# ESandML/SSL4GIE

Measured on AMD Instinct MI355X. Metric: images/sec/GPU (fwd+bwd) ViT-B 224² bs=256 at 1/2/4/8 MI355X; % MFMA peak, higher is better.
Workload: dtype bf16; 1 GPU; ViT-B MAE pretrain (mae_vit_base_patch16, norm_pix_loss, mask 0.75) fwd+bwd+grad-allreduce+AdamW, 224x224 synthetic N(0,1) images resident in HBM; batch_per_gpu=256, global_batch=256, parallelism=dp1, optimizer=AdamW(0.9,0.95) wd 0.05 (ssl4gie_amd.optim.ArenaAdamW)

## Files before the change

### include/ssl4gie_hip.h

```cpp
#ifndef SSL4GIE_HIP_H
#define SSL4GIE_HIP_H
#include <stddef.h>
#include <stdint.h>
#ifdef __cplusplus
extern "C" {
#endif

#define SSL4GIE_F32 0
#define SSL4GIE_BF16 1
#define SSL4GIE_EARG 1000
#define SSL4GIE_EPEER 1001

int ssl4gie_abi_version(void);

int ssl4gie_layernorm_fwd(const float* x, const float* gamma, const float* beta, void* y,
                          int y_dtype, float* mean, float* rstd, int rows, int cols, float eps,
                          void* stream);
size_t ssl4gie_layernorm_bwd_workspace_bytes(int rows, int cols);
int ssl4gie_layernorm_bwd(const void* dy, int dy_dtype, const float* x, const float* gamma,
                          const float* mean, const float* rstd, const float* dres, float* dx,
                          void* dx_lp, int lp_dtype, float* dgamma, float* dbeta, int accumulate,
                          float* workspace, int rows, int cols, void* stream);

size_t ssl4gie_colsum_workspace_bytes(int rows, int cols);
// ... 246 lines not shown
int ssl4gie_maxpool3x3s2_fwd(const void* x, void* y, unsigned char* arg, int dtype, int B, int H,
                             int W, int C, void* stream);
int ssl4gie_maxpool3x3s2_bwd(const void* dy, const unsigned char* arg, void* dx, int dtype, int B,
                             int H, int W, int C, void* stream);
int ssl4gie_bn_maxpool3x3s2_fwd(const void* x, const float* coef, int relu, void* y, unsigned char* arg,
                                int dtype, int B, int H, int W, int C, void* stream);
int ssl4gie_avgpool_fwd(const void* x, float* y, int dtype, int B, int HW, int C, void* stream);
int ssl4gie_avgpool_bwd(const float* dy, void* dx, int dtype, int B, int HW, int C, void* stream);

int ssl4gie_adamw_arena(float* p, const float* g, float* m, float* v, const long long* seg_start,
                        const float* seg_lr, const float* seg_wd, int S, float beta1, float beta2,
                        float eps, int step, long long n, void* stream);
int ssl4gie_adamw_arena_lp(float* p, const float* g, float* m, float* v, const long long* seg_start,
                           const float* seg_lr, const float* seg_wd, int S, float beta1, float beta2,
                           float eps, int step, long long n, void* lp_bf16, void* stream);
int ssl4gie_adamw_arena_range(float* p, const float* g, float* m, float* v, const long long* seg_start,
                              const float* seg_lr, const float* seg_wd, int S, float beta1, float beta2,
                              float eps, int step, long long lo, long long hi, void* lp_bf16,
                              void* stream);
size_t ssl4gie_grad_norm_workspace_bytes(void);
int ssl4gie_grad_norm_arena(const float* g, const long long* seg_start, const float* seg_mask, int S,
                            float inv_scale, float max_norm, void* workspace, float* ctl, long long n,
                            void* stream);
int ssl4gie_grad_scale_arena(float* g, const long long* seg_start, const float* seg_mask, int S,
                             const float* ctl, long long n, void* stream);
int ssl4gie_adamw_arena_range_ctl(float* p, const float* g, float* m, float* v, const long long* seg_start,
                                  const float* seg_lr, const float* seg_wd, int S, float beta1, float beta2,
                                  float eps, int* applied, long long lo, long long hi, void* lp_bf16,
                                  const float* ctl, int skip_nonfinite, int advance, void* stream);
size_t ssl4gie_lars_workspace_bytes(int S);
// ... 157 lines not shown
```

### ssl4gie_amd/_lib.py

```python
from __future__ import annotations

import ctypes as C
import os

_HERE = os.path.dirname(os.path.abspath(__file__))
LIB_PATH = os.path.join(_HERE, "libssl4gie_hip.so")
ABI_VERSION = 12

PROF_KINDS = 7

F32, BF16 = 0, 1
BWD_ACCUMULATE, BWD_NO_JOIN = 1, 4
EPI_NONE, EPI_BIAS, EPI_BIAS_GELU, EPI_BIAS_RESIDUAL, EPI_DGELU, EPI_BIAS_GELU_GRAD, EPI_MUL_AUX, \
    EPI_RELU_MASK_AUX, EPI_ADD_AUX, EPI_AFFINE_AUX_RELU = range(10)
BN_FROM_X, BN_FROM_PARTIALS, BN_FROM_STATS, BN_FROM_COEF = range(4)
FILTER_BILINEAR, FILTER_BICUBIC = 0, 1
TGT_U8, TGT_U16, TGT_F32 = range(3)
DET_MAP_MAX_PER_IMAGE, DET_MAP_CLASSES, DET_MAP_CHUNK = 1024, 256, 256
NMS_MAX_PER_SEGMENT = 4096
PRED_I64 = 2
ERASE_CONST, ERASE_RAND, ERASE_PIXEL = range(3)
BN_MASK_NONE, BN_MASK_Y, BN_MASK_X, BN_MASK_BITS = range(4)

vp, i32, i64, f32, sz = C.c_void_p, C.c_int, C.c_longlong, C.c_float, C.c_size_t
# ... 104 lines not shown
    "ssl4gie_bn_workspace_bytes": (sz, [i64, i32]),
    "ssl4gie_bn_fwd": (i32, [i32, vp, vp, i32, vp, vp, vp, vp, vp, vp, vp, vp, vp, vp, f32, f32, i32, vp, i32, i64, i32,
                             vp]),
    "ssl4gie_bn_stats": (i32, [vp, vp, i32, vp, vp, vp, i32, i64, i32, vp]),
    "ssl4gie_bn_bwd": (i32, [vp, i32, vp, vp, vp, vp, vp, vp, vp, vp, vp, vp, i32, vp, i32, i64, i32, vp]),
    "ssl4gie_bn_bwd_reduce": (i32, [vp, i32, vp, vp, vp, vp, vp, vp, vp, vp, vp, i32, i64, i32, vp]),
    "ssl4gie_bn_bwd_apply": (i32, [vp, i32, vp, vp, vp, vp, vp, vp, vp, f32, vp, vp, i32, i64, i32, vp]),
    "ssl4gie_ema_update": (i32, [vp, vp, f32, i64, vp]),
    "ssl4gie_maxpool3x3s2_fwd": (i32, [vp, vp, vp, i32, i32, i32, i32, i32, vp]),
    "ssl4gie_bn_maxpool3x3s2_fwd": (i32, [vp, vp, i32, vp, vp, i32, i32, i32, i32, i32, vp]),
    "ssl4gie_maxpool3x3s2_bwd": (i32, [vp, vp, vp, i32, i32, i32, i32, i32, vp]),
    "ssl4gie_avgpool_fwd": (i32, [vp, vp, i32, i32, i32, i32, vp]),
    "ssl4gie_avgpool_bwd": (i32, [vp, vp, i32, i32, i32, i32, vp]),
    "ssl4gie_adamw_arena": (i32, [vp, vp, vp, vp, vp, vp, vp, i32, f32, f32, f32, i32, i64, vp]),
    "ssl4gie_adamw_arena_lp": (i32, [vp, vp, vp, vp, vp, vp, vp, i32, f32, f32, f32, i32, i64, vp, vp]),
    "ssl4gie_adamw_arena_range": (i32, [vp, vp, vp, vp, vp, vp, vp, i32, f32, f32, f32, i32, i64, i64, vp, vp]),
    "ssl4gie_adamw_arena_range_ctl": (i32, [vp, vp, vp, vp, vp, vp, vp, i32, f32, f32, f32, vp, i64, i64, vp, vp,
                                            i32, i32, vp]),
    "ssl4gie_grad_norm_workspace_bytes": (sz, []),
    "ssl4gie_grad_norm_arena": (i32, [vp, vp, vp, i32, f32, f32, vp, vp, i64, vp]),
    "ssl4gie_grad_scale_arena": (i32, [vp, vp, vp, i32, vp, i64, vp]),
    "ssl4gie_lars_workspace_bytes": (sz, [i32]),
    "ssl4gie_lars_arena": (i32, [vp, vp, vp, vp, vp, vp, vp, i32, f32, f32, vp, i64, vp]),
    "ssl4gie_normalize_u8": (i32, [vp, vp, C.POINTER(C.c_float), C.POINTER(C.c_float), i32, i32, i32, vp]),
    "ssl4gie_view_sample_u8": (i32, [vp, i64, i32, i32, vp, vp, vp, vp, i32, i32, i32, C.POINTER(C.c_float),
                                     C.POINTER(C.c_float), vp]),
    "ssl4gie_quantize_u8": (i32, [vp, vp, i32, i32, vp]),
    "ssl4gie_randaug_layer_workspace_bytes": (sz, [i32]),
    "ssl4gie_randaug_layer": (i32, [vp, vp, vp, vp, vp, C.POINTER(C.c_ubyte), vp, i32, i32, vp]),
    "ssl4gie_normalize_erase_u8": (i32, [vp, vp, C.POINTER(C.c_float), C.POINTER(C.c_float), vp, i32, C.c_ulonglong, i32,
# ... 129 lines not shown
```

### ssl4gie_amd/csrc/engine.hip

```cpp
#include "common.h"
#include "ssl4gie_hip.h"

#include <string.h>
#include <stdlib.h>
#include <mutex>
#include "prof.h"
#include "internal.h"

extern "C" int ssl4gie_abi_version(void) { return 12; }

namespace { extern int g_wgrad_stream; }
extern "C" int ssl4gie_set_wgrad_stream(int on) {
    g_wgrad_stream = on ? 1 : 0;
    return 0;
}

ProfState g_prof = {false, 0, 0, nullptr, nullptr, nullptr};

extern "C" int ssl4gie_prof_begin(int max_launches) {
    REQUIRE(max_launches > 0 && !g_prof.ev);
    g_prof.ev = (hipEvent_t*)calloc((size_t)2 * max_launches, sizeof(hipEvent_t));
    g_prof.kind = (int*)calloc(max_launches, sizeof(int));
    g_prof.flops = (double*)calloc(max_launches, sizeof(double));
    REQUIRE(g_prof.ev && g_prof.kind && g_prof.flops);
// ... 292 lines not shown
    RC(linear_bwd_data(du, w->wfc1, w->wfc1_t, T, F, D, dt, e, stream));
    const bool ln_side = ss != nullptr;
    RC(ssl4gie_layernorm_bwd(dh, dt, a->xmid, w->ln2_g, a->mean2, a->rstd2, dx_out, dxmid,
                             (dt == SSL4GIE_F32 || s_attn) ? nullptr : dxmid_lp, dt, ln_side ? nullptr : g->ln2_g,
                             ln_side ? nullptr : g->ln2_b, accumulate, ln_ws, T, D, stream));
    if (s_attn) {
        RC(ssl4gie_drop_path_scale_cast(dxmid, s_attn, ws + P.dys_mid, dt, d->B, per_sample, stream));
        dxmid_lp = ws + P.dys_mid;
    }
    memset(&e, 0, sizeof(e));
    e.C = dattn; e.ldc = D; e.dtype_c = dt; e.epilogue = SSL4GIE_EPI_NONE;
    RC(linear_bwd_data(dxmid_lp, w->wproj, w->wproj_t, T, D, D, dt, e, stream));
    RC(ssl4gie_attn_bwd(a->qkv, a->attn, dattn, a->lse, dqkv, dt, d->B, d->N, d->H, D / d->H,
                        ws + L.attn_ws, stream));
    RC(fork());
    if (ln_side)
        RC(ssl4gie_internal_ln_reduce(ln_ws, g->ln2_g, g->ln2_b, T, D, accumulate, (hipStream_t)wst));
    wg = wgrad_desc(D, D, T, dxmid_lp, a->attn, g->wproj, g->bproj, dt, accumulate);
    wg2 = wgrad_desc(3 * D, D, T, dqkv, a->h1, g->wqkv, g->bqkv, dt, accumulate);
    RC(ssl4gie_gemm_tn_pair(&wg, &wg2, gws, L.gemm_ws_bytes, wst));
    memset(&e, 0, sizeof(e));
    e.C = dh; e.ldc = D; e.dtype_c = dt; e.epilogue = SSL4GIE_EPI_NONE;
    RC(linear_bwd_data(dqkv, w->wqkv, w->wqkv_t, T, 3 * D, D, dt, e, stream));
    RC(ssl4gie_layernorm_bwd(dh, dt, x_in, w->ln1_g, a->mean1, a->rstd1, dxmid, dx_in,
                             dt == SSL4GIE_F32 ? nullptr : dx_in_lp, dt, ln_side ? nullptr : g->ln1_g,
                             ln_side ? nullptr : g->ln1_b, accumulate, ln_side ? ln_ws1 : ln_ws, T, D, stream));
    if (ln_side) {
        RC(fork());
        RC(ssl4gie_internal_ln_reduce(ln_ws1, g->ln1_g, g->ln1_b, T, D, accumulate, ss->s));
    }
    if (ss && no_join) {
        HIP_RET(hipEventRecord(ss->ev[5 + slot], ss->s));
        ss->slot_used[slot] = true;
    } else if (ss) {
        HIP_RET(hipEventRecord(ss->ev[4], ss->s));
// ... 32 lines not shown
```

### ssl4gie_amd/csrc/gemm.hip

```cpp
#include "gemm_internal.h"

#include <mutex>
#include "prof.h"
#include <stdlib.h>

struct GemmArgs {
    int M, N, K, batch2;
    const void* A;
    long long sAm, sAk, sAb1, sAb2;
    const void* B;
    long long sBk, sBn, sBb1, sBb2;
    void* C;
    long long ldc, sCb1, sCb2;
    EpiArgs e;
};

template <typename TC, bool VEC, bool FAST = false>
DEVI void epi_store4(const EpiArgs& e, TC* __restrict__ C, long long ldc, int m, int n, int M,
                     int N, f32x4 acc) {
    if (m >= M || n >= N) return;
    const size_t off = (size_t)m * ldc + n;
    if (VEC) {
        f32x4 v = acc * e.alpha;
        switch (e.mode) {
// ... 583 lines not shown
        compute(cur);
    }

    float* out = (splits == 1) ? C : slabs + (size_t)split * M * N;
    const long long ldo = (splits == 1) ? ldc : N;
    EpiArgs es = e;
    if (splits != 1) { es.mode = SSL4GIE_EPI_NONE; es.accumulate = 0; es.alpha = 1.f; }
    epi_wave_tile<float, SSL4GIE_EPI_NONE>(es, out, ldo, m0 + wm, n0 + wn, M, N, acc, lane);
}

__global__ void slab_reduce_kernel(const float* __restrict__ slabs, float* __restrict__ C,
                                   long long ldc, int M, int N, int splits, float alpha,
                                   int accumulate, const float* __restrict__ cs_part,
                                   float* __restrict__ cs_out, unsigned c_blocks) {
    if (blockIdx.x >= c_blocks) {
        const int m = (blockIdx.x - c_blocks) * blockDim.x + threadIdx.x;
        if (m < M) {
            float s = 0.f;
            for (int k = 0; k < splits; ++k) s += cs_part[(size_t)k * M + m];
            cs_out[m] = accumulate ? cs_out[m] + s : s;
        }
        return;
    }
    const size_t i4 = (size_t)blockIdx.x * blockDim.x + threadIdx.x;
    const size_t total4 = (size_t)M * N / 4;
    if (i4 >= total4) return;
    const size_t idx = i4 * 4;
    const int m = (int)(idx / N), n = (int)(idx % N);
    f32x4 s = ld4(slabs + idx);
    int k = 1;
    for (; k + 3 < splits; k += 4) {
        const f32x4 a = ld4(slabs + (size_t)k * M * N + idx), b = ld4(slabs + (size_t)(k + 1) * M * N + idx);
        const f32x4 c2 = ld4(slabs + (size_t)(k + 2) * M * N + idx), d2 = ld4(slabs + (size_t)(k + 3) * M * N + idx);
        s += a; s += b; s += c2; s += d2;
    }
    for (; k < splits; ++k) s += ld4(slabs + (size_t)k * M * N + idx);
    s *= alpha;
    float* c = C + (size_t)m * ldc + n;
    if (accumulate) s += ld4(c);
    st4(c, s);
}

template <int G>
__global__ __launch_bounds__(64 * G) void slab_reduce_wide_kernel(const float* __restrict__ slabs,
                                                                  float* __restrict__ C, long long ldc, int M, int N,
                                                                  int splits, float alpha, int accumulate) {
    __shared__ f32x4 part[G - 1][64];
    const int c = threadIdx.x & 63, g = threadIdx.x >> 6;
    const size_t i4 = (size_t)blockIdx.x * 64 + c;
    const size_t total4 = (size_t)M * N / 4;
    const bool ok = i4 < total4;
    const size_t idx = i4 * 4, slab = (size_t)M * N;
    f32x4 s = {0, 0, 0, 0};
    if (ok)
    {
// ... 270 lines not shown
};
static TnManyPlan tn_many_plan(const ssl4gie_gemm_desc* ds, int n, int splits) {
    TnManyPlan p;
    size_t o = 0;
    for (int i = 0; i < n; ++i) {
        p.slab_off[i] = o;
        if (splits > 1) o += align256((size_t)splits * ds[i].M * ds[i].N * sizeof(float));
    }
    for (int i = 0; i < n; ++i) {
        p.cs_off[i] = o;
        if (splits > 1 && ds[i].colsum_a) o += align256((size_t)splits * ds[i].M * sizeof(float));
    }
    p.total = o;
    return p;
}
static int tn_many_run(const ssl4gie_gemm_desc* ds, int n, int splits, void* workspace, size_t workspace_bytes,
                       hipStream_t st) {
    for (int i = 0; i < n; ++i) {
        REQUIRE(ds[i].A && ds[i].B && ds[i].C);
        REQUIRE(!ds[i].colsum_a || ds[i].sAk >= ds[i].M);
    }
    const TnManyPlan p = tn_many_plan(ds, n, splits);
    REQUIRE(p.total == 0 || (workspace && workspace_bytes >= p.total));
    char* ws = (char*)workspace;
    float* slabs[TN_GROUP_MAX];
    float* cs[TN_GROUP_MAX];
    double flops = 0;
    for (int i = 0; i < n; ++i) {
        slabs[i] = splits > 1 ? (float*)(ws + p.slab_off[i]) : nullptr;
        cs[i] = (splits > 1 && ds[i].colsum_a) ? (float*)(ws + p.cs_off[i]) : nullptr;
        flops += 2.0 * ds[i].K * (double)ds[i].M * ds[i].N;
    }
    {
        ProfScope prof(PROF_GEMM_TN, flops, st);
        const int rc = ssl4gie_internal_tn256_launch(ds, n, splits, slabs, cs, st);
        if (rc) return rc;
    }
    for (int i = 0; splits > 1 && i < n; ++i) {
        const ssl4gie_gemm_desc* d = &ds[i];
        const int rc = launch_slab_reduce(slabs[i], (float*)d->C, d->ldc, d->M, d->N, splits, d->alpha, d->accumulate,
                                          cs[i], d->colsum_a, d->colsum_a != nullptr, false, st);
        if (rc) return rc;
    }
    return 0;
}

static bool tn_pair_ok(const ssl4gie_gemm_desc* a, const ssl4gie_gemm_desc* b) {
    return a && b && !nt_ok(a) && !nt_ok(b) && tn_ok(a) && tn_ok(b) && !a->conv && !b->conv &&
           ssl4gie_internal_tn256_ok(a) && ssl4gie_internal_tn256_ok(b) && a->K == b->K &&
           a->accumulate == b->accumulate && a->alpha == 1.f && b->alpha == 1.f &&
           a->N % 4 == 0 && b->N % 4 == 0;
}
extern "C" size_t ssl4gie_gemm_tn_pair_workspace_bytes(const ssl4gie_gemm_desc* a,
                                                       const ssl4gie_gemm_desc* b) {
    if (!a || !b) return 0;
    if (tn_pair_ok(a, b)) {
        const ssl4gie_gemm_desc ds[2] = {*a, *b};
// ... 1 lines not shown
    }
    const size_t wa = ssl4gie_gemm_workspace_bytes(a), wb = ssl4gie_gemm_workspace_bytes(b);
    return wa > wb ? wa : wb;
}
extern "C" int ssl4gie_gemm_tn_pair(const ssl4gie_gemm_desc* a, const ssl4gie_gemm_desc* b,
                                    void* workspace, size_t workspace_bytes, void* stream) {
    REQUIRE(a && b);
    if (!tn_pair_ok(a, b)) {
        const int rc = ssl4gie_gemm(a, workspace, workspace_bytes, stream);
        if (rc) return rc;
        return ssl4gie_gemm(b, workspace, workspace_bytes, stream);
    }
    const ssl4gie_gemm_desc ds[2] = {*a, *b};
    return tn_many_run(ds, 2, ssl4gie_internal_tn256_splits(ds, 2, TN_SPLIT_PAIR), workspace, workspace_bytes,
                       (hipStream_t)stream);
}

static bool tn_group_ok(const ssl4gie_gemm_desc* ds, int n) {
    if (!ds || n < 1 || n > TN_GROUP_MAX) return false;
    for (int i = 0; i < n; ++i) {
        const ssl4gie_gemm_desc* d = &ds[i];
        if (nt_ok(d) || !tn_ok(d) || d->conv || !ssl4gie_internal_tn256_ok(d) || d->K != ds[0].K ||
            d->N % 4 != 0 || d->dtype_c != SSL4GIE_F32)
            return false;
    }
    return true;
}
extern "C" size_t ssl4gie_gemm_tn_group_workspace_bytes(const ssl4gie_gemm_desc* descs, int n) {
    if (!descs || n < 1) return 0;
    if (tn_group_ok(descs, n))
// ... 22 lines not shown
```

### ssl4gie_amd/csrc/internal.h

```cpp
#pragma once
#include <hip/hip_runtime.h>
#include <stddef.h>

int ssl4gie_internal_reduce_partials(const float* partial, float* out, int nparts, int n_out,
                                     size_t stride, int accumulate, hipStream_t st);

int ssl4gie_internal_ln_reduce(const float* workspace, float* dgamma, float* dbeta, int rows, int cols,
                               int accumulate, hipStream_t st);
```

### ssl4gie_amd/csrc/norm.hip

```cpp
#include "common.h"
#include "prof.h"
#include "ssl4gie_hip.h"
#include "internal.h"

int ssl4gie_internal_compute_cus();

#define LN_ROWS_PER_BLOCK 4
#define LN_MAX_VEC 8

template <int NV> DEVI int ln_col(int i, int lane, int cols) {
    const int c = (i * 64 + lane) * 4;
    return (NV <= 4 && i < NV - 1) || c < cols ? c : 0;
}

static constexpr int ln_fwd_per_cu(int nv) { return nv == 1 ? 8 : nv == 2 ? 6 : nv == 3 ? 5 : nv == 4 ? 4 : 2; }
template <typename TY, int NV>
__global__ __launch_bounds__(256, ln_fwd_per_cu(NV)) void ln_fwd_kernel(const float* __restrict__ x,
                                                     const float* __restrict__ gamma,
                                                     const float* __restrict__ beta,
                                                     TY* __restrict__ y, float* __restrict__ mean,
                                                     float* __restrict__ rstd, int rows, int cols,
                                                     float eps) {
    const int lane = threadIdx.x & 63;
    const int stride = gridDim.x * LN_ROWS_PER_BLOCK;
// ... 303 lines not shown
                f32x4 og = ag[i], ob = ab[i];
#pragma unroll
                for (int w = 0; w < 3; ++w)
#pragma unroll
                    for (int j = 0; j < 4; ++j) {
                        og[j] += red[w][(i * 4 + j) * 64 + lane];
                        ob[j] += red[w][(NV * 4 + i * 4 + j) * 64 + lane];
                    }
                st4(pg + c, og);
                st4(pb + c, ob);
            }
        }
    }
}

#define RP_WAVES 16
__global__ __launch_bounds__(64 * RP_WAVES) void reduce_partials_kernel(
    const float* __restrict__ partial, float* __restrict__ out0, float* __restrict__ out1,
    int split, int nparts, int n_out, size_t stride, int accumulate) {
    __shared__ float red[RP_WAVES][64];
    const int lane = threadIdx.x & 63, wave = threadIdx.x >> 6;
    const int c = blockIdx.x * 64 + lane;
    float s0 = 0.f, s1 = 0.f, s2 = 0.f, s3 = 0.f;
    if (c < n_out) {
        int p = wave;
        for (; p + 15 * RP_WAVES < nparts; p += 16 * RP_WAVES) {
            float a[16];
#pragma unroll
            for (int u = 0; u < 16; ++u) a[u] = partial[(size_t)(p + u * RP_WAVES) * stride + c];
#pragma unroll
            for (int u = 0; u < 16; u += 4) { s0 += a[u]; s1 += a[u + 1]; s2 += a[u + 2]; s3 += a[u + 3]; }
        }
        for (; p + 3 * RP_WAVES < nparts; p += 4 * RP_WAVES) {
            s0 += partial[(size_t)p * stride + c];
            s1 += partial[(size_t)(p + RP_WAVES) * stride + c];
            s2 += partial[(size_t)(p + 2 * RP_WAVES) * stride + c];
            s3 += partial[(size_t)(p + 3 * RP_WAVES) * stride + c];
        }
        for (; p < nparts; p += RP_WAVES) s0 += partial[(size_t)p * stride + c];
    }
    red[wave][lane] = (s0 + s1) + (s2 + s3);
    __syncthreads();
    if (wave == 0 && c < n_out) {
        float s = 0.f;
#pragma unroll
        for (int w = 0; w < RP_WAVES; ++w) s += red[w][lane];
        float* o = (c < split) ? out0 + c : out1 + (c - split);
        *o = accumulate ? *o + s : s;
    }
}

template <typename T>
__global__ __launch_bounds__(256) void colsum_partial_kernel(const T* __restrict__ x,
                                                             float* __restrict__ partial,
                                                             int rows, int cols, size_t ld) {
    __shared__ f32x4 red[3][64];
    const int lane = threadIdx.x & 63, wave = threadIdx.x >> 6;
    const int c = (blockIdx.x * 64 + lane) * 4;
    f32x4 acc = {0, 0, 0, 0};
    if (c < cols) {
        for (int r = blockIdx.y * 4 + wave; r < rows; r += gridDim.y * 4) {
            const f32x4 v = ld4(x + (size_t)r * ld + c);
            acc += v;
        }
// ... 144 lines not shown
    }
#undef LN_BWD
#undef LN_BWD_RES
    LAUNCH_CHECK();
    if (dgamma && dbeta) {
        hipLaunchKernelGGL(reduce_partials_kernel, dim3((2 * cols + 63) / 64), dim3(64 * RP_WAVES),
                           0, st, workspace, dgamma, dbeta, cols, nb, 2 * cols, (size_t)2 * cols,
                           accumulate);
        LAUNCH_CHECK();
    }
    return 0;
}

int ssl4gie_internal_ln_reduce(const float* workspace, float* dgamma, float* dbeta, int rows, int cols,
                               int accumulate, hipStream_t st) {
    if (rows == 0 || !dgamma || !dbeta) return 0;
    const int nb = ln_bwd_blocks(rows);
    hipLaunchKernelGGL(reduce_partials_kernel, dim3((2 * cols + 63) / 64), dim3(64 * RP_WAVES), 0, st, workspace,
                       dgamma, dbeta, cols, nb, 2 * cols, (size_t)2 * cols, accumulate);
    LAUNCH_CHECK();
    return 0;
}

static bool colsum_narrow(int cols) { return cols <= 128 && cols % 4 == 0 && ((cols / 4) & (cols / 4 - 1)) == 0; }
static int colsum_parts(int rows, int cols) {
    const int cap = colsum_narrow(cols) ? 2048 : 256;
    int p = (rows + 63) / 64;
    return p < cap ? (p < 1 ? 1 : p) : cap;
}
extern "C" size_t ssl4gie_colsum_workspace_bytes(int rows, int cols) {
    return (size_t)colsum_parts(rows, cols) * cols * sizeof(float);
}
extern "C" int ssl4gie_colsum(const void* x, int dtype, float* out, int accumulate,
                              float* workspace, int rows, int cols, long long ld, void* stream) {
    REQUIRE(x && out && workspace && rows >= 0 && cols > 0 && ld >= cols);
    REQUIRE(dtype == SSL4GIE_F32 || dtype == SSL4GIE_BF16);
// ... 30 lines not shown
```

### ssl4gie_amd/csrc/optim_ops.hip

```cpp
#include "reduce.h"
#include "ssl4gie_hip.h"

namespace {
DEVI int find_seg(const long long* __restrict__ seg_start, int S, long long i) {
    int lo = 0, hi = S;
    while (hi - lo > 1) {
        const int mid = (lo + hi) >> 1;
        if (seg_start[mid] <= i) lo = mid;
        else hi = mid;
    }
    return lo;
}
DEVI int block_seg(const long long* __restrict__ seg_start, int S, long long i, long long block_first) {
    __shared__ int s0;
    if (threadIdx.x == 0) s0 = find_seg(seg_start, S, block_first);
    __syncthreads();
    int s = s0;
    while (s + 1 < S && seg_start[s + 1] <= i) ++s;
    return s;
}
}

template <bool CTL>
__global__ __launch_bounds__(256) void adamw_arena_kernel(
    float* __restrict__ p, const float* __restrict__ g, float* __restrict__ m, float* __restrict__ v,
    const long long* __restrict__ seg_start, const float* __restrict__ seg_lr,
    const float* __restrict__ seg_wd, int S, float b1, float b2, float eps, float bc1, float rsqrt_bc2,
    long long n, bf16_t* __restrict__ lp, long long lo, const float* __restrict__ ctl,
    const int* __restrict__ applied, int skip) {
    __shared__ float bc[2];
    float coef = 1.f;
    if (CTL) {
        if (skip && ctl[2] != 0.f) return;
        coef = ctl[1];
// ... 18 lines not shown
#pragma unroll
    for (int j = 0; j < 4; ++j) {
        float x = pp[j] * (1.f - lr * wd);
        const float mj = b1 * mm[j] + (1.f - b1) * gg[j];
        const float vj = b2 * vv[j] + (1.f - b2) * gg[j] * gg[j];
        x -= step * mj / (sqrtf(vj) * rsqrt_bc2 + eps);
        pp[j] = x; mm[j] = mj; vv[j] = vj;
    }
    st4(p + i, pp);
    st4(m + i, mm);
    st4(v + i, vv);
    if (lp) st4(lp + i, pp);
}
__global__ void adamw_advance_kernel(int* __restrict__ applied, const float* __restrict__ ctl, int skip) {
    if (!(skip && ctl[2] != 0.f)) *applied += 1;
}

#define GN_BLOCKS 2048
__global__ __launch_bounds__(256) void grad_norm_partial_kernel(
    const float* __restrict__ g, const long long* __restrict__ seg_start,
    const float* __restrict__ seg_mask, int S, float inv_scale, long long n, long long per_block,
    double* __restrict__ part_sum, int* __restrict__ part_bad) {
    __shared__ double red[4];
    __shared__ int redb[4];
    f32x4 acc = {0.f, 0.f, 0.f, 0.f};
    unsigned bad = 0;
    const long long lo = (long long)blockIdx.x * per_block;
    const long long hi = lo + per_block < n ? lo + per_block : n;
    long long i = lo + threadIdx.x * 4;
    if (i < hi) {
// ... 212 lines not shown
                                        const float* ctl, long long n, void* stream) {
    REQUIRE(g && seg_start && seg_mask && S > 0 && ctl && n > 0 && n % 4 == 0);
    hipLaunchKernelGGL(grad_scale_kernel, dim3((unsigned)((n / 4 + 255) / 256)), dim3(256), 0,
                       (hipStream_t)stream, g, seg_start, seg_mask, S, ctl, n);
    LAUNCH_CHECK();
    return 0;
}
extern "C" int ssl4gie_adamw_arena_lp(float* p, const float* g, float* m, float* v,
                                      const long long* seg_start, const float* seg_lr,
                                      const float* seg_wd, int S, float beta1, float beta2, float eps,
                                      int step, long long n, void* lp_bf16, void* stream) {
    REQUIRE(n >= 0);
    return ssl4gie_adamw_arena_range(p, g, m, v, seg_start, seg_lr, seg_wd, S, beta1, beta2, eps, step, 0, n,
                                     lp_bf16, stream);
}
extern "C" int ssl4gie_adamw_arena(float* p, const float* g, float* m, float* v,
                                   const long long* seg_start, const float* seg_lr,
                                   const float* seg_wd, int S, float beta1, float beta2, float eps,
                                   int step, long long n, void* stream) {
    return ssl4gie_adamw_arena_lp(p, g, m, v, seg_start, seg_lr, seg_wd, S, beta1, beta2, eps, step, n,
                                  nullptr, stream);
}
extern "C" size_t ssl4gie_lars_workspace_bytes(int S) {
    return ((size_t)S * LARS_PARTS * 2 + S) * sizeof(float);
}
extern "C" int ssl4gie_lars_arena(float* p, const float* g, float* mu, const long long* seg_start,
                                  const float* seg_lr, const float* seg_wd, const float* seg_mat, int S,
                                  float momentum, float trust, float* workspace, long long n,
                                  void* stream) {
    REQUIRE(p && g && mu && seg_start && seg_lr && seg_wd && seg_mat && workspace && S > 0 && S <= 65535 &&
// ... 17 lines not shown
```

### ssl4gie_amd/engine.py

```python
from __future__ import annotations

import ctypes as C
import contextlib
import os
import weakref
from dataclasses import dataclass
from typing import Callable, List, Optional, Sequence

import torch
import torch.nn as nn

from . import _lib, ops
from ._lib import BlockAct, BlockDims, BlockGrads, BlockWeights


def default_dtype():
    v = os.environ.get("SSL4GIE_PRECISION", "bf16").lower()
    return torch.float32 if v in ("fp32", "f32", "float32") else torch.bfloat16


def _align(n, a=256):
    return (n + a - 1) // a * a


# ... 60 lines not shown
        if getattr(self, "_lp_stamp", None) != weights_epoch():
            self._refresh_lp()
        o = self._index[id(p)]
        rows = p.shape[0]
        cols = p.numel() // rows
        return (self._lp[o:o + p.numel()].view(rows, cols), self._lpt[o:o + p.numel()].view(cols, rows))

    def lp_flat_for_update(self):
        if getattr(self, "_lp_stamp", None) != weights_epoch():
            self._refresh_lp()
        return self._lp

    def lp_flat_is_current(self):
        self._lp_flat_stamp = weights_epoch()
        self._lp_flat_versions = [p._version for p in self.params]

    def _refresh_lp(self):
        L = _lib.load()
        if getattr(self, "_lp", None) is None:
            self._lp = torch.empty(self.numel, dtype=torch.bfloat16, device=self.device)
            self._lpt = torch.zeros(self.numel, dtype=torch.bfloat16, device=self.device)
            mats = [(o, p.shape[0], p.numel() // p.shape[0]) for p, o in zip(self.params, self.offsets)
                    if p.ndim >= 2]
            starts = [0]
            for _, r, c in mats:
                starts.append(starts[-1] + ((r + 63) // 64) * ((c + 63) // 64))
            dev = self.device
            self._lp_tab = (torch.tensor([m[0] for m in mats], dtype=torch.int64, device=dev),
                            torch.tensor([m[1] for m in mats], dtype=torch.int32, device=dev),
                            torch.tensor([m[2] for m in mats], dtype=torch.int32, device=dev),
# ... 764 lines not shown
```

### ssl4gie_amd/optim.py

```python
from __future__ import annotations

import ctypes as C

import torch

from . import _lib
from .engine import ParamArena, bump_weights_epoch
from .ops import ptr, stream


def _adopt_grads(a, params):
    base, index = a.grad.data_ptr(), a._index
    for p in params:
        g = p.grad
        if g is not None and g.data_ptr() != base + 4 * index[id(p)]:
            v = a.grad_view(p)
            v.copy_(g)
            p.grad = v


class _GradNorm:

    def __init__(self, dev):
        L = _lib.load()
# ... 275 lines not shown
        ctl_path = clip_grad is not None or skip_nonfinite
        if ctl_path and self._overlap:
            raise ValueError("ArenaAdamW(overlap_backward=True) applies updates while the backward pass is "
                             "still running; clip_grad / skip_nonfinite need the norm of EVERY gradient first")
        a = self._arena()
        if self.exp_avg is None or self.exp_avg.numel() != a.numel:
            self.exp_avg = torch.zeros_like(a.data)
            self.exp_avg_sq = torch.zeros_like(a.data)
        key_before = self._tables_key
        tables = self._build_tables(a)
        if self._done and self._tables_key != key_before:
            raise RuntimeError("ArenaAdamW(overlap_backward=True): the set of parameters with gradients "
                               "changed between steps after part of this step was already applied")
        self._tables = tables
        self._lp = a.lp_flat_for_update() if a.data.is_cuda else None
        if ctl_path or self._dev_steps is not None:
            assert not self._done, "in-backward updates and the device-side step count do not mix"
            self._step_ctl(a, clip_grad, skip_nonfinite)
        else:
            st = stream()
            pos = 0
            for lo, hi in sorted(self._done) + [(a.numel, a.numel)]:
                if lo > pos:
                    self._launch(a, pos, lo, st)
                pos = max(pos, hi)
            if self._done:
                torch.cuda.current_stream(a.data.device).wait_stream(self._stream)
            self.step_count += 1
        self._done, self._seen, self._tables = [], {}, None
        bump_weights_epoch(touched=[p for g in self.param_groups for p in g["params"]])
        if self._lp is not None:
            a.lp_flat_is_current()


class ArenaLARS(_ArenaOptimizer):

    def __init__(self, model, params, lr=0.0, weight_decay=0.0, momentum=0.9, trust_coefficient=0.001):
        super().__init__(model, params, dict(lr=lr, weight_decay=weight_decay))
        self.momentum, self.trust = momentum, trust_coefficient
        self.mu = None
        self._ws = None

    def _state_buffers(self):
        return {"mu": self.mu}

    @torch.no_grad()
    def step(self):
# ... 14 lines not shown
```

Baseline: 11690 images/sec.

## Fuse AdamW with transposed bf16 weight emit; fold LN grad reduce into GEMM slab reduce

Adds an AdamW kernel that updates each weight matrix tile-wise and writes both the bf16 copy and a transposed bf16 copy through shared memory. This removes the separate pass that rebuilt transposed low-precision weights after each step. In the backward pass, the LayerNorm dgamma/dbeta partial reduction now rides inside a single multi-job reduce kernel together with the split-K slab reductions of the weight-gradient GEMM pair, cutting kernel launches. The cost is a more complex tiled optimizer kernel, plus a dependence on the lp table bookkeeping being consistent.

```diff
diff --git a/include/ssl4gie_hip.h b/include/ssl4gie_hip.h
--- a/include/ssl4gie_hip.h
+++ b/include/ssl4gie_hip.h
@@ -284,6 +284,11 @@
 int ssl4gie_adamw_arena_lp(float* p, const float* g, float* m, float* v, const long long* seg_start,
                            const float* seg_lr, const float* seg_wd, int S, float beta1, float beta2,
                            float eps, int step, long long n, void* lp_bf16, void* stream);
+int ssl4gie_adamw_arena_lpt(float* p, const float* g, float* m, float* v, const long long* seg_start,
+                            const float* seg_lr, const float* seg_wd, const float* seg_mat, int S, float beta1,
+                            float beta2, float eps, int step, long long n, void* lp_bf16, void* lpt_bf16,
+                            const long long* mat_off, const int* mat_rows, const int* mat_cols,
+                            const int* tile_start, int n_mats, int total_tiles, void* stream);
 int ssl4gie_adamw_arena_range(float* p, const float* g, float* m, float* v, const long long* seg_start,
                               const float* seg_lr, const float* seg_wd, int S, float beta1, float beta2,
                               float eps, int step, long long lo, long long hi, void* lp_bf16,
diff --git a/ssl4gie_amd/_lib.py b/ssl4gie_amd/_lib.py
--- a/ssl4gie_amd/_lib.py
+++ b/ssl4gie_amd/_lib.py
@@ -142,6 +142,8 @@
     "ssl4gie_avgpool_bwd": (i32, [vp, vp, i32, i32, i32, i32, vp]),
     "ssl4gie_adamw_arena": (i32, [vp, vp, vp, vp, vp, vp, vp, i32, f32, f32, f32, i32, i64, vp]),
     "ssl4gie_adamw_arena_lp": (i32, [vp, vp, vp, vp, vp, vp, vp, i32, f32, f32, f32, i32, i64, vp, vp]),
+    "ssl4gie_adamw_arena_lpt": (i32, [vp, vp, vp, vp, vp, vp, vp, vp, i32, f32, f32, f32, i32, i64, vp, vp, vp, vp, vp,
+                                      vp, i32, i32, vp]),
     "ssl4gie_adamw_arena_range": (i32, [vp, vp, vp, vp, vp, vp, vp, i32, f32, f32, f32, i32, i64, i64, vp, vp]),
     "ssl4gie_adamw_arena_range_ctl": (i32, [vp, vp, vp, vp, vp, vp, vp, i32, f32, f32, f32, vp, i64, i64, vp, vp,
                                             i32, i32, vp]),
diff --git a/ssl4gie_amd/csrc/engine.hip b/ssl4gie_amd/csrc/engine.hip
--- a/ssl4gie_amd/csrc/engine.hip
+++ b/ssl4gie_amd/csrc/engine.hip
@@ -330,11 +330,10 @@
     RC(ssl4gie_attn_bwd(a->qkv, a->attn, dattn, a->lse, dqkv, dt, d->B, d->N, d->H, D / d->H,
                         ws + L.attn_ws, stream));
     RC(fork());
-    if (ln_side)
-        RC(ssl4gie_internal_ln_reduce(ln_ws, g->ln2_g, g->ln2_b, T, D, accumulate, (hipStream_t)wst));
     wg = wgrad_desc(D, D, T, dxmid_lp, a->attn, g->wproj, g->bproj, dt, accumulate);
     wg2 = wgrad_desc(3 * D, D, T, dqkv, a->h1, g->wqkv, g->bqkv, dt, accumulate);
-    RC(ssl4gie_gemm_tn_pair(&wg, &wg2, gws, L.gemm_ws_bytes, wst));
+    const PartialsJob ln2 = ssl4gie_internal_ln_reduce_job(ln_ws, g->ln2_g, g->ln2_b, T, D, accumulate);
+    RC(ssl4gie_internal_gemm_tn_pair_riders(&wg, &wg2, gws, L.gemm_ws_bytes, &ln2, ln_side ? 1 : 0, (hipStream_t)wst));
     memset(&e, 0, sizeof(e));
     e.C = dh; e.ldc = D; e.dtype_c = dt; e.epilogue = SSL4GIE_EPI_NONE;
     RC(linear_bwd_data(dqkv, w->wqkv, w->wqkv_t, T, 3 * D, D, dt, e, stream));
diff --git a/ssl4gie_amd/csrc/gemm.hip b/ssl4gie_amd/csrc/gemm.hip
--- a/ssl4gie_amd/csrc/gemm.hip
+++ b/ssl4gie_amd/csrc/gemm.hip
@@ -1,4 +1,6 @@
 #include "gemm_internal.h"
+#include "internal.h"
+#include "reduce_jobs.h"
 
 #include <mutex>
 #include "prof.h"
@@ -621,31 +623,54 @@
                                    int accumulate, const float* __restrict__ cs_part,
                                    float* __restrict__ cs_out, unsigned c_blocks) {
     if (blockIdx.x >= c_blocks) {
-        const int m = (blockIdx.x - c_blocks) * blockDim.x + threadIdx.x;
-        if (m < M) {
-            float s = 0.f;
-            for (int k = 0; k < splits; ++k) s += cs_part[(size_t)k * M + m];
-            cs_out[m] = accumulate ? cs_out[m] + s : s;
-        }
+        slab_reduce_colsum(cs_part, cs_out, M, splits, accumulate, (blockIdx.x - c_blocks) * blockDim.x + threadIdx.x);
         return;
     }
-    const size_t i4 = (size_t)blockIdx.x * blockDim.x + threadIdx.x;
-    const size_t total4 = (size_t)M * N / 4;
-    if (i4 >= total4) return;
-    const size_t idx = i4 * 4;
-    const int m = (int)(idx / N), n = (int)(idx % N);
-    f32x4 s = ld4(slabs + idx);
-    int k = 1;
-    for (; k + 3 < splits; k += 4) {
-        const f32x4 a = ld4(slabs + (size_t)k * M * N + idx), b = ld4(slabs + (size_t)(k + 1) * M * N + idx);
-        const f32x4 c2 = ld4(slabs + (size_t)(k + 2) * M * N + idx), d2 = ld4(slabs + (size_t)(k + 3) * M * N + idx);
-        s += a; s += b; s += c2; s += d2;
-    }
-    for (; k < splits; ++k) s += ld4(slabs + (size_t)k * M * N + idx);
-    s *= alpha;
-    float* c = C + (size_t)m * ldc + n;
-    if (accumulate) s += ld4(c);
-    st4(c, s);
+    slab_reduce_c4(slabs, C, ldc, M, N, splits, alpha, accumulate, (size_t)blockIdx.x * blockDim.x + threadIdx.x);
+}
+
+#define REDUCE_JOBS_THREADS (64 * RP_WAVES)
+#define REDUCE_RIDERS_MAX 2
+struct SlabJob {
+    const float* slabs; float* C; long long ldc;
+    const float* cs_part; float* cs_out;
+    int M, N; float alpha; int accumulate;
+    unsigned blk0, c_blocks;
+};
+struct RiderJob {
+    const float* partial; float* out0; float* out1; size_t stride;
+    int split, nparts, n_out, accumulate;
+    unsigned blk0;
+};
+struct ReduceJobs {
+    int n_slab, n_rider, splits;
+    RiderJob r[REDUCE_RIDERS_MAX];
+    SlabJob s[TN_GROUP_MAX];
+};
+__global__ __launch_bounds__(REDUCE_JOBS_THREADS) void reduce_jobs_kernel(ReduceJobs J) {
+    __shared__ float red[RP_WAVES][64];
+    const unsigned b = blockIdx.x;
+    if (J.n_slab == 0 || b < J.s[0].blk0) {
+        RiderJob r = J.r[0];
+#pragma unroll
+        for (int i = 1; i < REDUCE_RIDERS_MAX; ++i)
+            if (i < J.n_rider && b >= J.r[i].blk0) r = J.r[i];
+        reduce_partials_strip(r.partial, r.out0, r.out1, r.split, r.nparts, r.n_out, r.stride, r.accumulate,
+                              (int)(b - r.blk0), red);
+        return;
+    }
+    SlabJob s = J.s[0];
+#pragma unroll
+    for (int i = 1; i < TN_GROUP_MAX; ++i)
+        if (i < J.n_slab && b >= J.s[i].blk0) s = J.s[i];
+    const unsigned rel = b - s.blk0;
+    if (rel >= s.c_blocks) {
+        slab_reduce_colsum(s.cs_part, s.cs_out, s.M, J.splits, s.accumulate,
+                           (int)((rel - s.c_blocks) * REDUCE_JOBS_THREADS + threadIdx.x));
+        return;
+    }
+    slab_reduce_c4(s.slabs, s.C, s.ldc, s.M, s.N, J.splits, s.alpha, s.accumulate,
+                   (size_t)rel * REDUCE_JOBS_THREADS + threadIdx.x);
 }
 
 template <int G>
@@ -946,8 +971,38 @@
     p.total = o;
     return p;
 }
+static int launch_reduce_jobs(const ssl4gie_gemm_desc* ds, int n, int splits, float* const* slabs, float* const* cs,
+                              const PartialsJob* riders, int n_riders, hipStream_t st) {
+    ReduceJobs J = {};
+    J.splits = splits;
+    unsigned blk = 0;
+    for (int i = 0; i < n_riders; ++i) {
+        const PartialsJob& p = riders[i];
+        if (p.n_out == 0) continue;
+        RiderJob& r = J.r[J.n_rider++];
+        r.partial = p.partial; r.out0 = p.out0; r.out1 = p.out1; r.stride = p.stride;
+        r.split = p.split; r.nparts = p.nparts; r.n_out = p.n_out; r.accumulate = p.accumulate;
+        r.blk0 = blk;
+        blk += (unsigned)((p.n_out + 63) / 64);
+    }
+    for (int i = 0; i < n; ++i) {
+        const ssl4gie_gemm_desc* d = &ds[i];
+        SlabJob& s = J.s[J.n_slab++];
+        const size_t total4 = (size_t)d->M * d->N / 4;
+        s.slabs = slabs[i]; s.C = (float*)d->C; s.ldc = d->ldc;
+        s.cs_part = cs[i]; s.cs_out = d->colsum_a;
+        s.M = d->M; s.N = d->N; s.alpha = d->alpha; s.accumulate = d->accumulate;
+        s.blk0 = blk;
+        s.c_blocks = (unsigned)((total4 + REDUCE_JOBS_THREADS - 1) / REDUCE_JOBS_THREADS);
+        blk += s.c_blocks + (d->colsum_a ? (unsigned)((d->M + REDUCE_JOBS_THREADS - 1) / REDUCE_JOBS_THREADS) : 0u);
+    }
+    hipLaunchKernelGGL(reduce_jobs_kernel, dim3(blk), dim3(REDUCE_JOBS_THREADS), 0, st, J);
+    LAUNCH_CHECK();
+    return 0;
+}
 static int tn_many_run(const ssl4gie_gemm_desc* ds, int n, int splits, void* workspace, size_t workspace_bytes,
-                       hipStream_t st) {
+                       hipStream_t st, const PartialsJob* riders = nullptr, int n_riders = 0) {
+    REQUIRE(n_riders >= 0 && n_riders <= REDUCE_RIDERS_MAX && (n_riders == 0 || riders));
     for (int i = 0; i < n; ++i) {
         REQUIRE(ds[i].A && ds[i].B && ds[i].C);
         REQUIRE(!ds[i].colsum_a || ds[i].sAk >= ds[i].M);
@@ -968,11 +1023,15 @@
         const int rc = ssl4gie_internal_tn256_launch(ds, n, splits, slabs, cs, st);
         if (rc) return rc;
     }
-    for (int i = 0; splits > 1 && i < n; ++i) {
-        const ssl4gie_gemm_desc* d = &ds[i];
-        const int rc = launch_slab_reduce(slabs[i], (float*)d->C, d->ldc, d->M, d->N, splits, d->alpha, d->accumulate,
-                                          cs[i], d->colsum_a, d->colsum_a != nullptr, false, st);
+    if (splits > 1 && (n > 1 || n_riders > 0)) return launch_reduce_jobs(ds, n, splits, slabs, cs, riders, n_riders, st);
+    for (int i = 0; i < n_riders; ++i) {
+        const int rc = ssl4gie_internal_reduce_partials_job(riders[i], st);
         if (rc) return rc;
+    }
+    if (splits > 1) {
+        const ssl4gie_gemm_desc* d = &ds[0];
+        return launch_slab_reduce(slabs[0], (float*)d->C, d->ldc, d->M, d->N, splits, d->alpha, d->accumulate, cs[0],
+                                  d->colsum_a, d->colsum_a != nullptr, false, st);
     }
     return 0;
 }
@@ -1004,6 +1063,21 @@
     const ssl4gie_gemm_desc ds[2] = {*a, *b};
     return tn_many_run(ds, 2, ssl4gie_internal_tn256_splits(ds, 2, TN_SPLIT_PAIR), workspace, workspace_bytes,
                        (hipStream_t)stream);
+}
+int ssl4gie_internal_gemm_tn_pair_riders(const ssl4gie_gemm_desc* a, const ssl4gie_gemm_desc* b, void* workspace,
+                                         size_t workspace_bytes, const PartialsJob* riders, int n_riders,
+                                         hipStream_t st) {
+    REQUIRE(a && b && n_riders >= 0 && n_riders <= REDUCE_RIDERS_MAX && (n_riders == 0 || riders));
+    if (!tn_pair_ok(a, b)) {
+        for (int i = 0; i < n_riders; ++i) {
+            const int rc = ssl4gie_internal_reduce_partials_job(riders[i], st);
+            if (rc) return rc;
+        }
+        return ssl4gie_gemm_tn_pair(a, b, workspace, workspace_bytes, st);
+    }
+    const ssl4gie_gemm_desc ds[2] = {*a, *b};
+    return tn_many_run(ds, 2, ssl4gie_internal_tn256_splits(ds, 2, TN_SPLIT_PAIR), workspace, workspace_bytes, st,
+                       riders, n_riders);
 }
 
 static bool tn_group_ok(const ssl4gie_gemm_desc* ds, int n) {
diff --git a/ssl4gie_amd/csrc/internal.h b/ssl4gie_amd/csrc/internal.h
--- a/ssl4gie_amd/csrc/internal.h
+++ b/ssl4gie_amd/csrc/internal.h
@@ -1,9 +1,21 @@
 #pragma once
 #include <hip/hip_runtime.h>
 #include <stddef.h>
+#include "ssl4gie_hip.h"
 
 int ssl4gie_internal_reduce_partials(const float* partial, float* out, int nparts, int n_out,
                                      size_t stride, int accumulate, hipStream_t st);
 
+struct PartialsJob {
+    const float* partial; float* out0; float* out1;
+    int split, nparts, n_out; size_t stride; int accumulate;
+};
+int ssl4gie_internal_reduce_partials_job(const PartialsJob& j, hipStream_t st);
+PartialsJob ssl4gie_internal_ln_reduce_job(const float* workspace, float* dgamma, float* dbeta, int rows, int cols,
+                                           int accumulate);
 int ssl4gie_internal_ln_reduce(const float* workspace, float* dgamma, float* dbeta, int rows, int cols,
                                int accumulate, hipStream_t st);
+
+int ssl4gie_internal_gemm_tn_pair_riders(const ssl4gie_gemm_desc* a, const ssl4gie_gemm_desc* b, void* workspace,
+                                         size_t workspace_bytes, const PartialsJob* riders, int n_riders,
+                                         hipStream_t st);
diff --git a/ssl4gie_amd/csrc/norm.hip b/ssl4gie_amd/csrc/norm.hip
--- a/ssl4gie_amd/csrc/norm.hip
+++ b/ssl4gie_amd/csrc/norm.hip
@@ -2,6 +2,7 @@
 #include "prof.h"
 #include "ssl4gie_hip.h"
 #include "internal.h"
+#include "reduce_jobs.h"
 
 int ssl4gie_internal_compute_cus();
 
@@ -341,40 +342,11 @@
     }
 }
 
-#define RP_WAVES 16
 __global__ __launch_bounds__(64 * RP_WAVES) void reduce_partials_kernel(
     const float* __restrict__ partial, float* __restrict__ out0, float* __restrict__ out1,
     int split, int nparts, int n_out, size_t stride, int accumulate) {
     __shared__ float red[RP_WAVES][64];
-    const int lane = threadIdx.x & 63, wave = threadIdx.x >> 6;
-    const int c = blockIdx.x * 64 + lane;
-    float s0 = 0.f, s1 = 0.f, s2 = 0.f, s3 = 0.f;
-    if (c < n_out) {
-        int p = wave;
-        for (; p + 15 * RP_WAVES < nparts; p += 16 * RP_WAVES) {
-            float a[16];
-#pragma unroll
-            for (int u = 0; u < 16; ++u) a[u] = partial[(size_t)(p + u * RP_WAVES) * stride + c];
-#pragma unroll
-            for (int u = 0; u < 16; u += 4) { s0 += a[u]; s1 += a[u + 1]; s2 += a[u + 2]; s3 += a[u + 3]; }
-        }
-        for (; p + 3 * RP_WAVES < nparts; p += 4 * RP_WAVES) {
-            s0 += partial[(size_t)p * stride + c];
-            s1 += partial[(size_t)(p + RP_WAVES) * stride + c];
-            s2 += partial[(size_t)(p + 2 * RP_WAVES) * stride + c];
-            s3 += partial[(size_t)(p + 3 * RP_WAVES) * stride + c];
-        }
-        for (; p < nparts; p += RP_WAVES) s0 += partial[(size_t)p * stride + c];
-    }
-    red[wave][lane] = (s0 + s1) + (s2 + s3);
-    __syncthreads();
-    if (wave == 0 && c < n_out) {
-        float s = 0.f;
-#pragma unroll
-        for (int w = 0; w < RP_WAVES; ++w) s += red[w][lane];
-        float* o = (c < split) ? out0 + c : out1 + (c - split);
-        *o = accumulate ? *o + s : s;
-    }
+    reduce_partials_strip(partial, out0, out1, split, nparts, n_out, stride, accumulate, blockIdx.x, red);
 }
 
 template <typename T>
@@ -549,12 +521,23 @@
 
 int ssl4gie_internal_ln_reduce(const float* workspace, float* dgamma, float* dbeta, int rows, int cols,
                                int accumulate, hipStream_t st) {
-    if (rows == 0 || !dgamma || !dbeta) return 0;
-    const int nb = ln_bwd_blocks(rows);
-    hipLaunchKernelGGL(reduce_partials_kernel, dim3((2 * cols + 63) / 64), dim3(64 * RP_WAVES), 0, st, workspace,
-                       dgamma, dbeta, cols, nb, 2 * cols, (size_t)2 * cols, accumulate);
+    return ssl4gie_internal_reduce_partials_job(
+        ssl4gie_internal_ln_reduce_job(workspace, dgamma, dbeta, rows, cols, accumulate), st);
+}
+int ssl4gie_internal_reduce_partials_job(const PartialsJob& j, hipStream_t st) {
+    if (j.n_out == 0) return 0;
+    hipLaunchKernelGGL(reduce_partials_kernel, dim3((j.n_out + 63) / 64), dim3(64 * RP_WAVES), 0, st, j.partial,
+                       j.out0, j.out1, j.split, j.nparts, j.n_out, j.stride, j.accumulate);
     LAUNCH_CHECK();
     return 0;
+}
+PartialsJob ssl4gie_internal_ln_reduce_job(const float* workspace, float* dgamma, float* dbeta, int rows, int cols,
+                                           int accumulate) {
+    PartialsJob j = {workspace, dgamma, dbeta, cols, 0, 0, (size_t)2 * cols, accumulate};
+    if (rows == 0 || !dgamma || !dbeta) return j;
+    j.nparts = ln_bwd_blocks(rows);
+    j.n_out = 2 * cols;
+    return j;
 }
 
 static bool colsum_narrow(int cols) { return cols <= 128 && cols % 4 == 0 && ((cols / 4) & (cols / 4 - 1)) == 0; }
diff --git a/ssl4gie_amd/csrc/optim_ops.hip b/ssl4gie_amd/csrc/optim_ops.hip
--- a/ssl4gie_amd/csrc/optim_ops.hip
+++ b/ssl4gie_amd/csrc/optim_ops.hip
@@ -18,6 +18,24 @@
     int s = s0;
     while (s + 1 < S && seg_start[s + 1] <= i) ++s;
     return s;
+}
+DEVI void adamw_elem(float& p, float& m, float& v, float g, float lr, float wd, float b1, float b2, float eps,
+                     float step, float rsqrt_bc2) {
+    const float decay = fmaf(-lr, wd, 1.f);
+    const float mj = fmaf(1.f - b1, g, b1 * m);
+    const float vj = fmaf(b2, v, ((1.f - b2) * g) * g);
+    const float q = (step * mj) / fmaf(sqrtf(vj), rsqrt_bc2, eps);
+    p = fmaf(p, decay, -q);
+    m = mj; v = vj;
+}
+DEVI void adamw_elem4(f32x4& p, f32x4& m, f32x4& v, const f32x4 g, float lr, float wd, float b1, float b2, float eps,
+                      float step, float rsqrt_bc2) {
+#pragma unroll
+    for (int j = 0; j < 4; ++j) {
+        float x = p[j], mj = m[j], vj = v[j];
+        adamw_elem(x, mj, vj, g[j], lr, wd, b1, b2, eps, step, rsqrt_bc2);
+        p[j] = x; m[j] = mj; v[j] = vj;
+    }
 }
 }
 
@@ -66,6 +84,111 @@
 }
 __global__ void adamw_advance_kernel(int* __restrict__ applied, const float* __restrict__ ctl, int skip) {
     if (!(skip && ctl[2] != 0.f)) *applied += 1;
+}
+
+__global__ __launch_bounds__(256) void adamw_arena_lpt_kernel(
+    float* __restrict__ p, const float* __restrict__ g, float* __restrict__ m, float* __restrict__ v,
+    const long long* __restrict__ seg_start, const float* __restrict__ seg_lr,
+    const float* __restrict__ seg_wd, const float* __restrict__ seg_mat, int S, float b1, float b2, float eps,
+    float bc1, float rsqrt_bc2, bf16_t* __restrict__ lp, bf16_t* __restrict__ lpt,
+    const long long* __restrict__ mat_off, const int* __restrict__ mat_rows, const int* __restrict__ mat_cols,
+    const int* __restrict__ tile_start, int n_mats, int total_tiles) {
+    __shared__ float tile[64][65];
+    __shared__ int sh_seg;
+    if ((int)blockIdx.x >= total_tiles) {
+        const int s = blockIdx.x - total_tiles;
+        const float lr = seg_lr[s];
+        if (lr < 0.f || seg_mat[s] != 0.f) return;
+        const float wd = seg_wd[s], step = lr / bc1;
+        const long long end = seg_start[s + 1];
+        for (long long i = seg_start[s] + threadIdx.x * 4; i < end; i += 1024) {
+            f32x4 pp = ld4(p + i), mm = ld4(m + i), vv = ld4(v + i);
+            const f32x4 gg = ld4(g + i);
+            adamw_elem4(pp, mm, vv, gg, lr, wd, b1, b2, eps, step, rsqrt_bc2);
+            st4(p + i, pp);
+            st4(m + i, mm);
+            st4(v + i, vv);
+            st4(lp + i, pp);
+        }
+        return;
+    }
+    const int t = blockIdx.x;
+    int lo = 0, hi = n_mats;
+    while (hi - lo > 1) {
+        const int mid = (lo + hi) >> 1;
+        if (tile_start[mid] <= t) lo = mid; else hi = mid;
+    }
+    const long long off = mat_off[lo];
+    if (threadIdx.x == 0) sh_seg = find_seg(seg_start, S, off);
+    __syncthreads();
+    const int s = sh_seg;
+    const float lr = seg_lr[s];
+    if (lr < 0.f) return;
+    const float wd = seg_wd[s], step = lr / bc1;
+    const int R = mat_rows[lo], Cc = mat_cols[lo], lt = t - tile_start[lo];
+    const int tiles_c = (Cc + 63) >> 6;
+    const int r0 = (lt / tiles_c) * 64, c0 = (lt % tiles_c) * 64;
+    const int tx = threadIdx.x & 15, ty = threadIdx.x >> 4;
+    const bool vec = (R % 4 == 0) && (Cc % 4 == 0);
+    const int c = c0 + 4 * tx;
+    if (vec) {
+        f32x4 pp[4], gg[4], mm[4], vv[4];
+#pragma unroll
+        for (int i = 0; i < 4; ++i) {
+            const int r = r0 + ty + 16 * i;
+            pp[i] = gg[i] = mm[i] = vv[i] = f32x4{0, 0, 0, 0};
+            if (r < R && c < Cc) {
+                const size_t e = (size_t)off + (size_t)r * Cc + c;
+                pp[i] = ld4(p + e); gg[i] = ld4(g + e); mm[i] = ld4(m + e); vv[i] = ld4(v + e);
+            }
+        }
+#pragma unroll
+        for (int i = 0; i < 4; ++i) {
+            const int r = r0 + ty + 16 * i;
+            if (r < R && c < Cc) {
+                const size_t e = (size_t)off + (size_t)r * Cc + c;
+                adamw_elem4(pp[i], mm[i], vv[i], gg[i], lr, wd, b1, b2, eps, step, rsqrt_bc2);
+                st4(p + e, pp[i]);
+                st4(m + e, mm[i]);
+                st4(v + e, vv[i]);
+                st4(lp + e, pp[i]);
+            }
+#pragma unroll
+            for (int j = 0; j < 4; ++j) tile[ty + 16 * i][4 * tx + j] = pp[i][j];
+        }
+    } else {
+#pragma unroll
+        for (int i = 0; i < 4; ++i) {
+            const int r = r0 + ty + 16 * i;
+#pragma unroll
+            for (int j = 0; j < 4; ++j) {
+                float x = 0.f;
+                if (r < R && c + j < Cc) {
+                    const size_t e = (size_t)off + (size_t)r * Cc + c + j;
+                    float mj = m[e], vj = v[e];
+                    x = p[e];
+                    adamw_elem(x, mj, vj, g[e], lr, wd, b1, b2, eps, step, rsqrt_bc2);
+                    p[e] = x; m[e] = mj; v[e] = vj;
+                    lp[e] = f2bf(x);
+                }
+                tile[ty + 16 * i][4 * tx + j] = x;
+            }
+        }
+    }
+    __syncthreads();
+    bf16_t* dp = lpt + off;
+#pragma unroll
+    for (int i = 0; i < 4; ++i) {
+        const int cc = c0 + ty + 16 * i, r = r0 + 4 * tx;
+        if (cc < Cc) {
+            const f32x4 o = {tile[4 * tx][ty + 16 * i], tile[4 * tx + 1][ty + 16 * i],
+                             tile[4 * tx + 2][ty + 16 * i], tile[4 * tx + 3][ty + 16 * i]};
+            if (vec && r + 3 < R) st4(dp + (size_t)cc * R + r, o);
+            else
+#pragma unroll
+                for (int j = 0; j < 4; ++j) if (r + j < R) dp[(size_t)cc * R + r + j] = f2bf(o[j]);
+        }
+    }
 }
 
 #define GN_BLOCKS 2048
@@ -308,6 +431,23 @@
     return ssl4gie_adamw_arena_range(p, g, m, v, seg_start, seg_lr, seg_wd, S, beta1, beta2, eps, step, 0, n,
                                      lp_bf16, stream);
 }
+extern "C" int ssl4gie_adamw_arena_lpt(float* p, const float* g, float* m, float* v, const long long* seg_start,
+                                       const float* seg_lr, const float* seg_wd, const float* seg_mat, int S,
+                                       float beta1, float beta2, float eps, int step, long long n, void* lp_bf16,
+                                       void* lpt_bf16, const long long* mat_off, const int* mat_rows,
+                                       const int* mat_cols, const int* tile_start, int n_mats, int total_tiles,
+                                       void* stream) {
+    REQUIRE(p && g && m && v && seg_start && seg_lr && seg_wd && seg_mat && S > 0 && step > 0 && n >= 0 && n % 4 == 0);
+    REQUIRE(lp_bf16 && lpt_bf16 && mat_off && mat_rows && mat_cols && tile_start && n_mats > 0 && total_tiles > 0);
+    if (n == 0) return 0;
+    const float bc1 = 1.f - powf(beta1, (float)step), bc2 = 1.f - powf(beta2, (float)step);
+    hipLaunchKernelGGL(adamw_arena_lpt_kernel, dim3((unsigned)total_tiles + (unsigned)S), dim3(256), 0,
+                       (hipStream_t)stream, p, g, m, v, seg_start, seg_lr, seg_wd, seg_mat, S, beta1, beta2, eps, bc1,
+                       1.f / sqrtf(bc2), (bf16_t*)lp_bf16, (bf16_t*)lpt_bf16, mat_off, mat_rows, mat_cols, tile_start,
+                       n_mats, total_tiles);
+    LAUNCH_CHECK();
+    return 0;
+}
 extern "C" int ssl4gie_adamw_arena(float* p, const float* g, float* m, float* v,
                                    const long long* seg_start, const float* seg_lr,
                                    const float* seg_wd, int S, float beta1, float beta2, float eps,
diff --git a/ssl4gie_amd/csrc/reduce_jobs.h b/ssl4gie_amd/csrc/reduce_jobs.h
--- /dev/null
+++ b/ssl4gie_amd/csrc/reduce_jobs.h
@@ -0,0 +1,66 @@
+#pragma once
+#include "common.h"
+
+DEVI void slab_reduce_c4(const float* __restrict__ slabs, float* __restrict__ C, long long ldc, int M, int N, int splits,
+                         float alpha, int accumulate, size_t i4) {
+    const size_t total4 = (size_t)M * N / 4;
+    if (i4 >= total4) return;
+    const size_t idx = i4 * 4;
+    const int m = (int)(idx / N), n = (int)(idx % N);
+    f32x4 s = ld4(slabs + idx);
+    int k = 1;
+    for (; k + 3 < splits; k += 4) {
+        const f32x4 a = ld4(slabs + (size_t)k * M * N + idx), b = ld4(slabs + (size_t)(k + 1) * M * N + idx);
+        const f32x4 c2 = ld4(slabs + (size_t)(k + 2) * M * N + idx), d2 = ld4(slabs + (size_t)(k + 3) * M * N + idx);
+        s += a; s += b; s += c2; s += d2;
+    }
+    for (; k < splits; ++k) s += ld4(slabs + (size_t)k * M * N + idx);
+    s *= alpha;
+    float* c = C + (size_t)m * ldc + n;
+    if (accumulate) s += ld4(c);
+    st4(c, s);
+}
+
+DEVI void slab_reduce_colsum(const float* __restrict__ cs_part, float* __restrict__ cs_out, int M, int splits,
+                             int accumulate, int m) {
+    if (m < M) {
+        float s = 0.f;
+        for (int k = 0; k < splits; ++k) s += cs_part[(size_t)k * M + m];
+        cs_out[m] = accumulate ? cs_out[m] + s : s;
+    }
+}
+
+#define RP_WAVES 16
+DEVI void reduce_partials_strip(const float* __restrict__ partial, float* __restrict__ out0, float* __restrict__ out1,
+                                int split, int nparts, int n_out, size_t stride, int accumulate, int strip,
+                                float (*red)[64] ) {
+    const int lane = threadIdx.x & 63, wave = threadIdx.x >> 6;
+    const int c = strip * 64 + lane;
+    float s0 = 0.f, s1 = 0.f, s2 = 0.f, s3 = 0.f;
+    if (c < n_out) {
+        int p = wave;
+        for (; p + 15 * RP_WAVES < nparts; p += 16 * RP_WAVES) {
+            float a[16];
+#pragma unroll
+            for (int u = 0; u < 16; ++u) a[u] = partial[(size_t)(p + u * RP_WAVES) * stride + c];
+#pragma unroll
+            for (int u = 0; u < 16; u += 4) { s0 += a[u]; s1 += a[u + 1]; s2 += a[u + 2]; s3 += a[u + 3]; }
+        }
+        for (; p + 3 * RP_WAVES < nparts; p += 4 * RP_WAVES) {
+            s0 += partial[(size_t)p * stride + c];
+            s1 += partial[(size_t)(p + RP_WAVES) * stride + c];
+            s2 += partial[(size_t)(p + 2 * RP_WAVES) * stride + c];
+            s3 += partial[(size_t)(p + 3 * RP_WAVES) * stride + c];
+        }
+        for (; p < nparts; p += RP_WAVES) s0 += partial[(size_t)p * stride + c];
+    }
+    red[wave][lane] = (s0 + s1) + (s2 + s3);
+    __syncthreads();
+    if (wave == 0 && c < n_out) {
+        float s = 0.f;
+#pragma unroll
+        for (int w = 0; w < RP_WAVES; ++w) s += red[w][lane];
+        float* o = (c < split) ? out0 + c : out1 + (c - split);
+        *o = accumulate ? *o + s : s;
+    }
+}
diff --git a/ssl4gie_amd/engine.py b/ssl4gie_amd/engine.py
--- a/ssl4gie_amd/engine.py
+++ b/ssl4gie_amd/engine.py
@@ -98,6 +98,12 @@
     def lp_flat_is_current(self):
         self._lp_flat_stamp = weights_epoch()
         self._lp_flat_versions = [p._version for p in self.params]
+
+    def lp_tables_for_update(self):
+        return ((self._lpt,) + self._lp_tab) if self._lp_tab[4] else None
+
+    def lp_all_current(self):
+        self._lp_stamp = weights_epoch()
 
     def _refresh_lp(self):
         L = _lib.load()
diff --git a/ssl4gie_amd/optim.py b/ssl4gie_amd/optim.py
--- a/ssl4gie_amd/optim.py
+++ b/ssl4gie_amd/optim.py
@@ -313,12 +313,22 @@
                                "changed between steps after part of this step was already applied")
         self._tables = tables
         self._lp = a.lp_flat_for_update() if a.data.is_cuda else None
+        lpt_written = False
         if ctl_path or self._dev_steps is not None:
             assert not self._done, "in-backward updates and the device-side step count do not mix"
             self._step_ctl(a, clip_grad, skip_nonfinite)
         else:
             st = stream()
             pos = 0
+            lpt = a.lp_tables_for_update() if (self._lp is not None and not self._done) else None
+            if lpt is not None:
+                start, lr, wd, mat, S = self._tables
+                _lib.check(_lib.load().ssl4gie_adamw_arena_lpt(
+                    ptr(a.data), ptr(a.grad), ptr(self.exp_avg), ptr(self.exp_avg_sq), ptr(start), ptr(lr), ptr(wd),
+                    ptr(mat), S, self.betas[0], self.betas[1], self.eps, self.step_count + 1, a.numel, ptr(self._lp),
+                    ptr(lpt[0]), ptr(lpt[1]), ptr(lpt[2]), ptr(lpt[3]), ptr(lpt[4]), lpt[5], lpt[6], st),
+                    "adamw_arena_lpt")
+                pos, lpt_written = a.numel, True
             for lo, hi in sorted(self._done) + [(a.numel, a.numel)]:
                 if lo > pos:
                     self._launch(a, pos, lo, st)
@@ -330,6 +340,8 @@
         bump_weights_epoch(touched=[p for g in self.param_groups for p in g["params"]])
         if self._lp is not None:
             a.lp_flat_is_current()
+            if lpt_written:
+                a.lp_all_current()
 
 
 class ArenaLARS(_ArenaOptimizer):
```

Result: no change. 11770 images/sec (median of 6 runs) (+0.7%).
